# MAPieschl/PointCloudProcessing

Measured on AMD Instinct MI355X. Metric: points/sec PointNet fwd+bwd N=1024 B=32 at 1/2/4/8 MI355X vs CPU ref, higher is better.
Workload: dtype bf16; 1 GPU; PointNet-cls training step (fwd + losses + bwd + grad all-reduce + Adam), N=1024 points, batch 32 per GPU, profile classification_pretrain, 23 classes / 12 parts, random-init weights; global_batch=32, points_per_cloud=1024, parallelism=dp1, launch=hipgraph

## Files before the change

include/pointnet_hip.h:

```cpp
#ifndef POINTNET_HIP_H
#define POINTNET_HIP_H

#include <stddef.h>
#include <stdint.h>

#ifdef __cplusplus
extern "C" {
#endif

#define PN_ABI_VERSION 6

typedef enum {
  PN_OK = 0,
  PN_ERR_INVALID_ARGUMENT = -1,
  PN_ERR_LAUNCH = -2,
  PN_ERR_UNSUPPORTED = -3,
  PN_ERR_WORKSPACE = -4
} pn_status;

#define PN_PREC_BF16 1
#define PN_PREC_BF16X3 3
#define PN_STORE_BF16 0x100
#define PN_IO_KEEP_ACTIVATIONS 1

// ... 25 lines not shown

int pn_conv_fwd_max(const pn_operand* x, const float* w, int B, int N, int K, int C, const float* sgn,
                    float* pmax, int32_t* pidx, float* stat_partials, int prec, pn_stream stream);

int pn_weights_prep(const float* w, const float* sgn, int K, int C, void* wf_hi, void* wf_lo, pn_stream stream);
int pn_panel_slots_per_cloud(int B, int N);
int pn_conv_fwd_max_panel(const pn_operand* x, const void* wf_hi, const void* wf_lo, int B, int N, int K, int C, float* pmax,
                          int32_t* pblock, float* sumsq, int64_t* colacc, int prec, pn_stream stream);
int pn_panel_finalize(const float* pmax, const int32_t* pblock, const float* sumsq, const int64_t* colacc, const void* wf_hi, const void* wf_lo,
                      int prec, int B, int N, int K, int C, const float* gamma, const float* beta, float* moving_mean, float* moving_var,
                      float momentum, float eps, int use_batch_stats, int update_moving, float* mean, float* invstd, float* scale, float* shift,
                      float* g, float* zstar, int32_t* arg_block, pn_stream stream);
int pn_chain_fwd_max(const pn_operand* x, const float* xyz, const float* w1, const void* w1t, const float* scale1, const float* shift1,
                     const void* w2t, const float* scale2, const float* shift2, const void* wf_hi, int B, int N, float* pmax,
                     int32_t* pblock, pn_stream stream);
int pn_weights_copy16(const float* w, int K, int C, void* w16, void* wt16, pn_stream stream);

int pn_max_resolve(const pn_operand* x, const void* wf_hi, const void* wf_lo, const int32_t* arg_block, int B, int N, int K, int C,
                   int32_t* arg, int prec, pn_stream stream);

int pn_maxbwd_scatter(const int32_t* arg, const float* hs, const float* wt, const float* q, int B, int N, int K, int C, float* D, int store16,
                      pn_stream stream);

int pn_conv_bwd_data(const pn_operand* dz, const float* w, int64_t w_cloud_stride, int B, int N, int K, int C,
                     const float* addend, const float* zmask, const float* msc, const float* msh, float* out,
                     float* stat_partials, int prec, pn_stream stream);

int pn_conv_bwd_data_wgrad(const pn_operand* dz, const float* w, int64_t w_cloud_stride, int B, int N, int K, int C,
                           const float* addend, const float* zmask, const float* msc, const float* msh, float* out,
                           float* stat_partials, const pn_operand* a, int Ci, int slab_rows, float* slabs, int prec, pn_stream stream);

int pn_conv_wgrad(const pn_operand* a, const pn_operand* b, int B, int N, int Ci, int Cj, int slab_rows,
                  float* slabs, int prec, pn_stream stream);

int pn_slab_reduce(const float* slabs, int n_slabs, int per_group, int64_t elems, float* out, pn_stream stream);

int pn_bn_finalize(const float* stat_partials, int n_tiles, int C, int64_t count, const float* gamma,
                   const float* beta, float* moving_mean, float* moving_var, float momentum, float eps,
                   int use_batch_stats, int update_moving, float* mean, float* invstd, float* scale, float* shift,
                   pn_stream stream);

int pn_bn_bwd_finalize(const float* stat_partials, int n_tiles, int C, int64_t count, const float* gamma,
                       const float* mean, const float* invstd, int batch_stats, float* dgamma, float* dbeta,
                       float* ca, float* cb, float* cc, pn_stream stream);

int pn_sign(const float* gamma, int C, float* sgn, pn_stream stream);

int pn_max_finalize(const float* pmax, const int32_t* pidx, int B, int tiles_per_cloud, int C, const float* sgn,
                    const float* scale, const float* shift, float* g, float* zstar, int32_t* arg, pn_stream stream);

size_t pn_dense_workspace_floats(int R, int K, int C);
int pn_dense_layer(const float* x, int ldx, const float* w, int ldw, int trans, int R, int K, int C, float* workspace,
                   uint32_t* counters, const float* bias, const float* gamma, const float* beta, float* moving_mean,
                   float* moving_var, float momentum, float eps, int bn_mode, int act, const uint8_t* keep, float keep_scale,
                   float* z_out, float* a_out, float* mean_out, float* invstd_out, pn_stream stream);

int pn_dense_bwd(const float* da, const float* z, const float* x, int ldx, int R, int K, int C, const float* gamma,
                 const float* beta, const float* mean, const float* invstd, int bn_mode, int act, const uint8_t* keep,
                 float keep_scale, float* dz, float* dgamma, float* dbeta, float* dbias, float* dw, pn_stream stream);

typedef struct pn_dense_tail {
  const float *z, *gamma, *beta, *mean, *invstd;
  const uint8_t* keep; float keep_scale;
  int bn_mode, act;
  float *dz, *dgamma, *dbeta, *dbias;
} pn_dense_tail;
// ... 218 lines not shown
```

pointcloudprocessing_amd/_lib.py:

```python
from __future__ import annotations

import ctypes as C
import os
import subprocess

_HERE = os.path.dirname(os.path.abspath(__file__))
LIB_PATH = os.path.join(_HERE, "libpointnet_hip.so")
CSRC = os.path.join(_HERE, "csrc")

PN_PREC_BF16 = 1
PN_PREC_BF16X3 = 3
PN_STORE_BF16 = 0x100
PN_IO_KEEP_ACTIVATIONS = 1
ABI_VERSION = 6
PN_NUM_BLOCKS = 15
PN_ICP_BVH_LEAF = 4
PN_ICP_BVH_MAX_DEPTH = 32
PN_ICP_BVH_PAD_ULPS = 16
PREC = {"bf16": PN_PREC_BF16 | PN_STORE_BF16, "bf16_f32act": PN_PREC_BF16, "bf16x3": PN_PREC_BF16X3}

BLOCK_NAMES = ["input_transform", "mlp_1_1", "mlp_1_2", "feature_transform", "mlp_2_1", "mlp_2_2", "mlp_2_3",
               "mlp_cls_1", "mlp_cls_2", "mlp_cls_3", "mlp_seg_1", "mlp_seg_2", "mlp_seg_3", "mlp_seg_4",
               "mlp_seg_5"]

# ... 40 lines not shown
                ("bwd_phase", C.c_int32), ("flags", C.c_int32), ("dropout_seed", C.c_uint64), ("dropout_step", C.c_void_p),
                ("sync_rank", C.c_int32), ("pad3_", C.c_int32), ("sync_hook", C.c_void_p), ("sync_ctx", C.c_void_p)]


SYNC_HOOK = C.CFUNCTYPE(C.c_int, C.c_void_p, C.c_int, C.c_void_p, C.c_void_p, C.c_int64, C.c_int, C.c_void_p)


_P = C.c_void_p
_I = C.c_int
_I64 = C.c_int64
_F = C.c_float
_D = C.c_double
_OP = C.POINTER(pn_operand)
_DESC = C.POINTER(pn_model_desc)
_IO = C.POINTER(pn_model_io)
SIGNATURES = {
    "pn_abi_version": (_I, []),
    "pn_last_error": (C.c_char_p, []),
    "pn_normalize": (_I, [_P, _I, _I, _P, _P, _P, _P]),
    "pn_conv3_fwd": (_I, [_P, _P, _I64, _I, _I, _I, _P, _P, _P]),
    "pn_conv3_wgrad": (_I, [_P, _OP, _I, _I, _I, _P, _P]),
    "pn_conv_fwd": (_I, [_OP, _P, _I64, _I, _I, _I, _I, _P, _P, _P, _I, _P]),
    "pn_conv_fwd_max": (_I, [_OP, _P, _I, _I, _I, _I, _P, _P, _P, _P, _I, _P]),
    "pn_weights_prep": (_I, [_P, _P, _I, _I, _P, _P, _P]),
    "pn_panel_slots_per_cloud": (_I, [_I, _I]),
    "pn_conv_fwd_max_panel": (_I, [_OP, _P, _P, _I, _I, _I, _I, _P, _P, _P, _P, _I, _P]),
    "pn_panel_finalize": (_I, [_P, _P, _P, _P, _P, _P, _I, _I, _I, _I, _I, _P, _P, _P, _P, _F, _F, _I, _I, _P, _P, _P, _P, _P, _P, _P, _P]),
    "pn_chain_fwd_max": (_I, [_OP, _P, _P, _P, _P, _P, _P, _P, _P, _P, _I, _I, _P, _P, _P]),
    "pn_weights_copy16": (_I, [_P, _I, _I, _P, _P, _P]),
    "pn_max_resolve": (_I, [_OP, _P, _P, _P, _I, _I, _I, _I, _P, _I, _P]),
    "pn_maxbwd_scatter": (_I, [_P, _P, _P, _P, _I, _I, _I, _I, _P, _I, _P]),
    "pn_conv_bwd_data": (_I, [_OP, _P, _I64, _I, _I, _I, _I, _P, _P, _P, _P, _P, _P, _I, _P]),
    "pn_conv_wgrad": (_I, [_OP, _OP, _I, _I, _I, _I, _I, _P, _I, _P]),
    "pn_conv_bwd_data_wgrad": (_I, [_OP, _P, _I64, _I, _I, _I, _I, _P, _P, _P, _P, _P, _P, _OP, _I, _I, _P, _I, _P]),
    "pn_slab_reduce": (_I, [_P, _I, _I, _I64, _P, _P]),
    "pn_bn_finalize": (_I, [_P, _I, _I, _I64, _P, _P, _P, _P, _F, _F, _I, _I, _P, _P, _P, _P, _P]),
    "pn_bn_bwd_finalize": (_I, [_P, _I, _I, _I64, _P, _P, _P, _I, _P, _P, _P, _P, _P, _P]),
    "pn_sign": (_I, [_P, _I, _P, _P]),
    "pn_max_finalize": (_I, [_P, _P, _I, _I, _I, _P, _P, _P, _P, _P, _P, _P]),
    "pn_dense_workspace_floats": (C.c_size_t, [_I, _I, _I]),
    "pn_dense_layer": (_I, [_P, _I, _P, _I, _I, _I, _I, _I, _P, _P, _P, _P, _P, _P, _P, _F, _F, _I, _I, _P, _F, _P, _P, _P, _P, _P]),
    "pn_dense_bwd_step": (_I, [_P, _I, _P, _I, _I, _I, _I, _P, _P, _P, _P, _P]),
    "pn_dense_wgrad_batch": (_I, [_P, _I, _P]),
    "pn_dense_bwd": (_I, [_P, _P, _P, _I, _I, _I, _I, _P, _P, _P, _P, _I, _I, _P, _F, _P, _P, _P, _P, _P, _P]),
    "pn_softmax_xent": (_I, [_P, _I, _I, _P, _F, _P, _P, _P, _P, _P]),
    "pn_argmax_rows": (_I, [_P, _I64, _I, _P, _P]),
    "pn_seg_out_part_stride": (_I, []),
    "pn_seg_out_part_rows": (_I, []),
    "pn_seg_out_fwd": (_I, [_OP, _P, _P, _I64, _I, _I, _P, _F, _P, _P, _P, _P]),
    "pn_bmm": (_I, [_P, _P, _I, _I, _I, _P, _I, _P]),
    "pn_dropout_masks": (_I, [_P, _I64, _P, _I64, _F, C.c_uint64, _P, _P]),
    "pn_count_nonfinite": (_I, [_P, _I64, _I, _P, _P]),
    "pn_fps_workspace_bytes": (C.c_size_t, [_I, _I]),
    "pn_fps": (_I, [_P, _I, _I, _I, _I, _P, _P, _P, C.c_size_t, _P]),
    "pn_voxel_workspace_bytes": (C.c_size_t, [_I]),
    "pn_voxel_downsample": (_I, [_P, _P, _I, C.POINTER(C.c_float), C.POINTER(C.c_float), _I, _P, _P, _P, _P, _P,
                                 C.c_size_t, _P]),
    "pn_knn_propagate": (_I, [_P, _P, _I, _I, _I, _I, _P, _I, _P, _P, _P, _P, _P]),
    "pn_icp_workspace_bytes": (C.c_size_t, [_I, _I, _I, _I]),
    "pn_icp_correspond": (_I, [_P, _P, _I, _I, _P, C.POINTER(C.c_int32), _I, _I, _P, _F, _P, _P, _P, _P, C.c_size_t, _P]),
    "pn_icp_solve": (_I, [_P, _I, _P, _P, _P, _P]),
    "pn_semantic_icp": (_I, [_P, _P, _I, _I, _P, C.POINTER(C.c_int32), _I, _I, _P, _I, _F, _D, _D, _P, _P, _P, _P, _P, _P,
                             C.c_size_t, _P]),
    "pn_icp_normals": (_I, [_P, C.POINTER(C.c_int32), _I, _I, _I, _P, _P, _P, _P]),
    "pn_icp_plane_workspace_bytes": (C.c_size_t, [_I, _I, _I, _I]),
    "pn_icp_plane_sums": (_I, [_P, _P, _I, _I, _P, C.POINTER(C.c_int32), _I, _I, _P, _F, _P, _P, _P, _P, _P, _P, C.c_size_t, _P]),
# ... 123 lines not shown
```

pointcloudprocessing_amd/csrc/pn_api.hip:

```cpp
#include <stdarg.h>
#include "pn_internal.h"

namespace pn {
static thread_local char g_err[512] = "";
void set_error(const char* fmt, ...) {
  va_list ap;
  va_start(ap, fmt);
  vsnprintf(g_err, sizeof(g_err), fmt, ap);
  va_end(ap);
}
const char* get_error() { return g_err; }
}

using namespace pn;
static inline hipStream_t S(pn_stream s) { return reinterpret_cast<hipStream_t>(s); }

extern "C" {

int pn_abi_version(void) { return PN_ABI_VERSION; }
const char* pn_last_error(void) { return get_error(); }

int pn_normalize(const float* xyz, int B, int N, float* out, float* centroid, float* scale, pn_stream stream) {
  return normalize(xyz, B, N, out, centroid, scale, S(stream));
}
// ... 25 lines not shown
                      float* g, float* zstar, int32_t* arg_block, pn_stream stream) {
  return panel_finalize(pmax, pblock, sumsq, reinterpret_cast<const long long*>(colacc), wf_hi, wf_lo, prec, B, N, K, C, gamma, beta, moving_mean, moving_var, momentum, eps,
                        use_batch_stats, update_moving, mean, invstd, scale, shift, g, zstar, arg_block, S(stream));
}
int pn_chain_fwd_max(const pn_operand* x, const float* xyz, const float* w1, const void* w1t, const float* scale1, const float* shift1,
                     const void* w2t, const float* scale2, const float* shift2, const void* wf_hi, int B, int N, float* pmax, int32_t* pblock,
                     pn_stream stream) {
  return chain_fwd_max(x, xyz, w1, w1t, scale1, shift1, w2t, scale2, shift2, wf_hi, B, N, pmax, pblock, S(stream));
}
int pn_weights_copy16(const float* w, int K, int C, void* w16, void* wt16, pn_stream stream) { return weights_copy16(w, K, C, w16, wt16, S(stream)); }
int pn_max_resolve(const pn_operand* x, const void* wf_hi, const void* wf_lo, const int32_t* arg_block, int B, int N, int K, int C,
                   int32_t* arg, int prec, pn_stream stream) {
  return max_resolve(x, wf_hi, wf_lo, prec, arg_block, B, N, K, C, arg, S(stream));
}
int pn_maxbwd_scatter(const int32_t* arg, const float* hs, const float* wt, const float* q, int B, int N, int K, int C, float* D, int store16,
                      pn_stream stream) {
  PN_CHECK_ARG(B > 0 && N > 0 && C > 0, "pn_maxbwd_scatter: bad sizes");
  return maxbwd_scatter(arg, hs, wt, q, B, N, K, C, D, store16, S(stream));
}
int pn_conv_bwd_data(const pn_operand* dz, const float* w, int64_t wcs, int B, int N, int K, int C, const float* addend,
                     const float* zmask, const float* msc, const float* msh, float* out, float* part, int prec, pn_stream stream) {
  return conv_bwd_data(dz, w, wcs, B, N, K, C, addend, zmask, msc, msh, out, part, prec, S(stream));
}
int pn_conv_bwd_data_wgrad(const pn_operand* dz, const float* w, int64_t wcs, int B, int N, int K, int C, const float* addend,
                           const float* zmask, const float* msc, const float* msh, float* out, float* part, const pn_operand* a, int Ci,
                           int slab_rows, float* slabs, int prec, pn_stream stream) {
  PN_CHECK_ARG(a != nullptr, "pn_conv_bwd_data_wgrad: null operand a");
  const WgradFuse wf{*a, Ci, slab_rows, slabs};
  return conv_bwd_data(dz, w, wcs, B, N, K, C, addend, zmask, msc, msh, out, part, prec, S(stream), nullptr, nullptr, &wf);
}
int pn_conv_wgrad(const pn_operand* a, const pn_operand* b, int B, int N, int Ci, int Cj, int slab_rows, float* slabs, int prec,
                  pn_stream stream) {
  return conv_wgrad(a, b, B, N, Ci, Cj, slab_rows, slabs, prec, S(stream));
}
int pn_slab_reduce(const float* slabs, int n_slabs, int per_group, int64_t elems, float* out, pn_stream stream) {
  return slab_reduce(slabs, n_slabs, per_group, elems, out, S(stream));
}
int pn_bn_finalize(const float* part, int n_tiles, int C, int64_t count, const float* gamma, const float* beta, float* mm, float* mv,
                   float momentum, float eps, int use_batch_stats, int update_moving, float* mean, float* invstd, float* scale,
                   float* shift, pn_stream stream) {
  return bn_finalize(part, n_tiles, C, count, gamma, beta, mm, mv, momentum, eps, use_batch_stats, update_moving, mean, invstd, scale,
                     shift, S(stream));
}
int pn_bn_bwd_finalize(const float* part, int n_tiles, int C, int64_t count, const float* gamma, const float* mean,
                       const float* invstd, int batch_stats, float* dgamma, float* dbeta, float* ca, float* cb, float* cc,
                       pn_stream stream) {
  return bn_bwd_finalize(part, n_tiles, C, count, gamma, mean, invstd, batch_stats, dgamma, dbeta, ca, cb, cc, S(stream));
}
int pn_sign(const float* gamma, int C, float* sgn, pn_stream stream) { return sign_of(gamma, C, sgn, S(stream)); }
int pn_max_finalize(const float* pmax, const int32_t* pidx, int B, int tpc, int C, const float* sgn, const float* scale,
                    const float* shift, float* g, float* zstar, int32_t* arg, pn_stream stream) {
  return max_finalize(pmax, pidx, B, tpc, C, 0x7fffffff, sgn, scale, shift, g, zstar, arg, S(stream));
}
size_t pn_dense_workspace_floats(int R, int K, int C) { return dense_partial_floats(R, K, C); }
int pn_dense_layer(const float* x, int ldx, const float* w, int ldw, int trans, int R, int K, int C, float* workspace, uint32_t* counters,
                   const float* bias, const float* gamma, const float* beta, float* moving_mean, float* moving_var, float momentum,
                   float eps, int bn_mode, int act, const uint8_t* keep, float keep_scale, float* z_out, float* a_out, float* mean_out,
                   float* invstd_out, pn_stream stream) {
  return dense_layer(x, ldx, w, ldw, trans != 0, R, K, C, workspace, counters, bias, gamma, beta, moving_mean, moving_var, momentum, eps,
                     bn_mode, act, keep, keep_scale, z_out, a_out, mean_out, invstd_out, S(stream));
}
int pn_dense_bwd(const float* da, const float* z, const float* x, int ldx, int R, int K, int C, const float* gamma, const float* beta,
                 const float* mean, const float* invstd, int bn_mode, int act, const uint8_t* keep, float keep_scale, float* dz,
                 float* dgamma, float* dbeta, float* dbias, float* dw, pn_stream stream) {
  if (R <= 32)
    return dense_bwd_fused(da, z, x, ldx, R, K, C, gamma, beta, mean, invstd, bn_mode, act, keep, keep_scale, dz, dgamma, dbeta, dbias, dw,
// ... 194 lines not shown
```

pointcloudprocessing_amd/csrc/pn_gemm.hip:

```cpp
#include <vector>
#include "pn_common.h"
#include "pn_dense_wgrad.h"
#include "pn_gemm_core.h"
#include "pn_internal.h"
#include "pn_slab_reduce.h"

namespace pn {

template <int BM, int BN, int NS, bool B2>
__global__ __launch_bounds__(256) void wgrad_batch_kernel(const WgradBatch wb) {
  __shared__ __attribute__((aligned(16))) unsigned char lds_raw[GemmLds<BM, BN, NS>::BYTES];
  wgrad_batch_tile<BM, BN, NS, B2>(wb, (int)blockIdx.x, lds_raw);
}

template <int BM, int BN, int NS, bool B2>
__global__ __launch_bounds__(256) void wgrad_batch_dense_kernel(const WgradBatch wb, int n_w, const DenseWgradBatch db) {
  __shared__ __attribute__((aligned(16))) unsigned char lds_raw[GemmLds<BM, BN, NS>::BYTES];
  static_assert(GemmLds<BM, BN, NS>::BYTES >= 16 * 32 * 4, "the dense riders' LDS tile fits");
  if ((int)blockIdx.x >= n_w) {
    dense_wgrad_batch_body(db, (int)blockIdx.x - n_w, reinterpret_cast<float(*)[32]>(lds_raw));
    return;
  }
  wgrad_batch_tile<BM, BN, NS, B2>(wb, (int)blockIdx.x, lds_raw);
}

struct WgLds {
  static constexpr int PITCH = Geo<64>::PITCH;
  static constexpr int W = 2 * 128 * PITCH, A = W + 64 * PITCH, RED_BYTES = (A + 128 * PITCH) * 2, BYTES = RED_BYTES + 4 * 64 * 4;
  static_assert(BYTES <= 65536, "the fused weight-gradient tile's LDS exceeds the static __shared__ limit");
};
template <int BM, int BN, int NS, int MODE, bool A2, int EPI, bool ADD, bool MASK, bool AH, bool S16, bool W16 = false, bool WG = false>
__device__ __forceinline__ void rows_tile_t(const GemmArgs& g, const int bx, const int by, unsigned char* lds_raw, const WgArgs* wa = nullptr) {
  constexpr int BK = (NS == 3) ? 32 : 64;
  constexpr int PITCH = Geo<BK>::PITCH;
  constexpr int MT = BM / 64, NT = BN / 64;
  constexpr int WTM = BM / 2, WTN = BN / 2;
  constexpr int TILE_A = BM * PITCH, TILE_B = BN * PITCH;
  static_assert(!WG || (BM == 128 && BN == 64 && NS == 1 && MODE == MODE_BWD && EPI == EPI_STORE && AH && S16), "the fused weight-gradient tile");
  __bf16* Ahi = reinterpret_cast<__bf16*>(lds_raw);
  __bf16* Bhi = Ahi + (WG ? WgLds::W : TILE_A);
  __bf16* Alo = (NS == 3) ? (Bhi + TILE_B) : Ahi;
  __bf16* Blo = (NS == 3) ? (Alo + TILE_A) : Bhi;

  const int tid = threadIdx.x, lane = tid & 63, wave = tid >> 6;
  const int wm = wave >> 1, wn = wave & 1;
  const int wrow0 = wm * WTM, wcol0 = wn * WTN;

  f32x16 acc[MT][NT];
#pragma unroll
  for (int m = 0; m < MT; ++m)
#pragma unroll
    for (int n = 0; n < NT; ++n)
#pragma unroll
      for (int e = 0; e < 16; ++e) acc[m][n][e] = 0.f;

  const int cloud = bx / g.tiles_per_cloud, tin = bx - cloud * g.tiles_per_cloud;

  const int row_in_cloud0 = tin * BM;
  const int nrows = min(BM, g.N - row_in_cloud0);
  const long long row0 = (long long)cloud * g.N + row_in_cloud0;
  const int col0 = by * BN;
  const long long wbase = (long long)cloud * g.w_cloud_stride;
  pn_operand wop;
  wop.s1 = g.w; wop.s2 = nullptr; wop.ca = nullptr; wop.cb = nullptr; wop.cc = nullptr;
  wop.lo = -INFINITY; wop.h16 = 0;
  wop.ld = (MODE == MODE_FWD) ? g.C : g.K;

  NatStage<BM, BK, A2, AH> sa;
  TrnStage<BN, BK, false, false> sbT;
  NatStage<BN, BK, false, false> sbN;
  CopyStage<BN, BK> sbC;
  auto issue_chunk = [&](int k0) {
    if (!(g.dbg & 4)) sa.issue(g.a, row0 * g.a.ld, nrows, k0, tid);
    if constexpr (W16) {
      sbC.issue(g.w16, (long long)col0 * g.K, g.K, g.C - col0, k0, tid);
    } else if (MODE == MODE_FWD) {
      if (!(g.dbg & 8)) sbT.issue(wop, wbase + (long long)k0 * g.C + col0, BK, g.C - col0, tid);
    } else {
      sbN.issue(wop, wbase + (long long)col0 * g.K, g.C - col0, k0, tid);
    }
  };
  NatStage<BM, BK, false, true> swg;
  if constexpr (WG) swg.issue(wa->a, row0 * wa->a.ld, nrows, 0, tid);
  if (g.K > 0) issue_chunk(0);
  for (int k0 = 0; k0 < g.K; k0 += BK) {
    sa.pin();
    if constexpr (WG) {
      Ahi = reinterpret_cast<__bf16*>(lds_raw) + (k0 / BK) * TILE_A;
      Alo = Ahi;
    }
    sa.template finish<NS>(Ahi, Alo, g.a, nrows, k0, tid);
    if constexpr (W16) {
      sbC.pin();
      sbC.finish(Bhi, g.C - col0, tid);
    } else if (MODE == MODE_FWD) {
      sbT.pin();
      sbT.template finish<NS>(Bhi, Blo, wop, BK, g.C - col0, 0, tid);
    } else {
      sbN.pin();
      sbN.template finish<NS>(Bhi, Blo, wop, g.C - col0, k0, tid);
    }
    __syncthreads();
    if (k0 + BK < g.K) issue_chunk(k0 + BK);
    mma_chunk<MT, NT, BK, NS>(acc, Ahi, Alo, Bhi, Blo, wrow0, wcol0, lane);
    __syncthreads();
  }
  if constexpr (WG) {
    swg.pin();
    swg.template finish<1>(reinterpret_cast<__bf16*>(lds_raw) + WgLds::A, reinterpret_cast<__bf16*>(lds_raw) + WgLds::A, wa->a, nrows, 0, tid);
  }

  const int r = lane & 31, h = lane >> 5;
  const bool full = (nrows == BM) && (col0 + BN <= g.C);
  float* red = reinterpret_cast<float*>(lds_raw + (WG ? WgLds::RED_BYTES : 0));

  if (EPI == EPI_STORE) {
    float s1[NT], s2[NT];
#pragma unroll
    for (int n = 0; n < NT; ++n) {
      const int jl = wcol0 + n * 32 + r, j = col0 + jl;
      const bool jv = j < g.C;
      float bias = 0.f, msc = 0.f, msh = 0.f;
      if (jv && g.cloud_bias) bias = g.cloud_bias[(long long)cloud * g.cloud_bias_stride + j];
      if (jv && g.zmask) { msc = g.msc[j]; msh = g.msh[j]; }
      float a1 = 0.f, a2 = 0.f;
#pragma unroll
      for (int m = 0; m < MT; ++m) {
        const int il0 = wrow0 + m * 32 + 4 * h;
        if (full) {
          if (g.out && !(g.dbg & 1)) epi_store_block<true, ADD, MASK, true, S16>(acc[m][n], g, row0, il0, nrows, j, jv, bias, msc, msh, a1, a2);
          else epi_store_block<true, ADD, MASK, false, S16>(acc[m][n], g, row0, il0, nrows, j, jv, bias, msc, msh, a1, a2);
        } else {
          if (g.out) epi_store_block<false, ADD, MASK, true, S16>(acc[m][n], g, row0, il0, nrows, j, jv, bias, msc, msh, a1, a2);
          else epi_store_block<false, ADD, MASK, false, S16>(acc[m][n], g, row0, il0, nrows, j, jv, bias, msc, msh, a1, a2);
        }
      }
      s1[n] = a1 + __shfl_xor(a1, 32, 64);
      s2[n] = a2 + __shfl_xor(a2, 32, 64);
// ... 92 lines not shown
    const int ncol = g.ncol;
    if (ncol > 1) {
      const int lin = blockIdx.x, nrow = (int)gridDim.x / ncol, full = (nrow / 8) * 8 * ncol;
      if (lin < full) {
        const int grp = lin / (8 * ncol), r = lin - grp * 8 * ncol;
        by = r >> 3;
        bx = grp * 8 + (r & 7);
      } else {
        const int l2 = lin - full, rem = nrow - (nrow / 8) * 8;
        bx = (nrow / 8) * 8 + l2 % rem;
        by = l2 / rem;
      }
    }
    if (g.a.h16) {
      if constexpr (NS == 1 && EPI == EPI_STORE) {
        if (g.w16) {
          if (g.store16) rows_tile_t<BM, BN, NS, MODE, A2, EPI, ADD, MASK, true, true, true>(g, bx, by, lds_raw);
          else rows_tile_t<BM, BN, NS, MODE, A2, EPI, ADD, MASK, true, false, true>(g, bx, by, lds_raw);
          return;
        }
      }
      if (EPI == EPI_STORE && g.store16) rows_tile_t<BM, BN, NS, MODE, A2, EPI, ADD, MASK, true, EPI == EPI_STORE>(g, bx, by, lds_raw);
      else rows_tile_t<BM, BN, NS, MODE, A2, EPI, ADD, MASK, true, false>(g, bx, by, lds_raw);
    } else {
      if (EPI == EPI_STORE && g.store16) rows_tile_t<BM, BN, NS, MODE, A2, EPI, ADD, MASK, false, EPI == EPI_STORE>(g, bx, by, lds_raw);
      else rows_tile_t<BM, BN, NS, MODE, A2, EPI, ADD, MASK, false, false>(g, bx, by, lds_raw);
    }
  }
}

template <bool ADD, bool MASK>
__global__ __launch_bounds__(256) void gemm_bwd_wgrad_kernel(const GemmArgs g, const WgArgs wa) {
  __shared__ __attribute__((aligned(16))) unsigned char lds_raw[WgLds::BYTES];
  if (g.w16) rows_tile_t<128, 64, 1, MODE_BWD, true, EPI_STORE, ADD, MASK, true, true, true, true>(g, (int)blockIdx.x, 0, lds_raw, &wa);
  else rows_tile_t<128, 64, 1, MODE_BWD, true, EPI_STORE, ADD, MASK, true, true, false, true>(g, (int)blockIdx.x, 0, lds_raw, &wa);
}

template <bool AH, bool S16>
__global__ __launch_bounds__(256) void gemm_bwd_reduce_kernel(const GemmArgs g, int n_gemm, const float* __restrict__ slabs, int per_group,
                                                              long long elems, float* __restrict__ red_out, int nb_per_group) {
  constexpr int LDS_BYTES = (128 + 64) * Geo<64>::PITCH * 2;
  static_assert(LDS_BYTES >= 8 * 32 * 4, "the riders' LDS tile fits");
  __shared__ __attribute__((aligned(16))) unsigned char lds_raw[LDS_BYTES];
  if ((int)blockIdx.x >= n_gemm) {
    const int bx = (int)blockIdx.x - n_gemm;
    slab_reduce_block(slabs, per_group, elems, red_out, bx % nb_per_group, bx / nb_per_group, reinterpret_cast<float(*)[32]>(lds_raw));
    return;
  }
  rows_tile_t<128, 64, 1, MODE_BWD, false, EPI_STORE, false, false, AH, S16>(g, (int)blockIdx.x, 0, lds_raw);
}

template <int BM, int BN, int NS, int MODE, bool A2, bool B2, int EPI, bool ADD = false, bool MASK = false>
static int launch(const GemmArgs& g, dim3 grid, hipStream_t st) {
  hipLaunchKernelGGL((gemm_kernel<BM, BN, NS, MODE, A2, B2, EPI, ADD, MASK>), grid, dim3(256), 0, st, g);
  PN_CHECK_LAUNCH();
  return PN_OK;
}

static bool aligned16(const void* p) { return (reinterpret_cast<uintptr_t>(p) & 15) == 0; }

static int check_operand(const pn_operand* o, const char* name) {
  PN_CHECK_ARG(o && o->s1, "%s: null operand", name);
  PN_CHECK_ARG(aligned16(o->s1) && (!o->s2 || aligned16(o->s2)), "%s: s1/s2 must be 16-byte aligned", name);
  PN_CHECK_ARG((!o->ca || aligned16(o->ca)) && (!o->cb || aligned16(o->cb)) && (!o->cc || aligned16(o->cc)),
               "%s: coefficient vectors must be 16-byte aligned", name);
  PN_CHECK_ARG(o->ld > 0 && o->ld % 4 == 0, "%s: ld must be a positive multiple of 4", name);
  PN_CHECK_ARG(o->h16 == 0 || (o->h16 == 1 && o->ld % 8 == 0), "%s: h16 must be 0 or 1, and 16-bit rows need ld %% 8 == 0", name);
  return PN_OK;
// ... 65 lines not shown
  PN_CHECK_ARG(K >= 64 && K % 64 == 0, "pn_conv_fwd_max: K must be a multiple of 64 (K=%d)", K);
  PN_CHECK_ARG(C >= 128 && C % 128 == 0, "pn_conv_fwd_max: C must be a multiple of 128 (C=%d)", C);
  PN_CHECK_ARG(x->ld >= K, "pn_conv_fwd_max: x.ld < K");
  PN_CHECK_ARG(w && aligned16(w) && sgn && pmax && pidx, "pn_conv_fwd_max: null pointer");
  PN_CHECK_ARG(prec == PN_PREC_BF16 || prec == PN_PREC_BF16X3, "pn_conv_fwd_max: bad prec %d", prec);
  GemmArgs g;
  memset(&g, 0, sizeof(g));
  g.a = *x; g.w = w; g.B = B; g.N = N; g.K = K; g.C = C;
  g.tiles_per_cloud = cdiv(N, 128);
  g.sgn = sgn; g.pmax = pmax; g.pidx = pidx; g.stat_partials = stat_partials;
  return dispatch_rows<MODE_FWD, false, EPI_MAX>(g, prec, st);
}

int conv_bwd_data(const pn_operand* dz, const float* w, long long wcs, int B, int N, int K, int C, const float* addend,
                  const float* zmask, const float* msc, const float* msh, float* out, float* stat_partials, int prec,
                  hipStream_t st, const void* w16, const float* col_bias, const WgradFuse* wf) {
  PN_TRY(check_operand(dz, "pn_conv_bwd_data.dz"));
  PN_CHECK_ARG(B > 0 && N > 0, "pn_conv_bwd_data: B and N must be positive");
  PN_CHECK_ARG(K >= 64 && K % 64 == 0, "pn_conv_bwd_data: K must be a multiple of 64 (K=%d)", K);
  PN_CHECK_ARG(C >= 64 && C % 64 == 0, "pn_conv_bwd_data: C must be a multiple of 64 (C=%d)", C);
  PN_CHECK_ARG(dz->ld >= K, "pn_conv_bwd_data: dz.ld < K");
  PN_CHECK_ARG(w && aligned16(w), "pn_conv_bwd_data: w null or unaligned");
  PN_CHECK_ARG(!zmask || (msc && msh), "pn_conv_bwd_data: zmask needs msc and msh");
  const int store16 = (prec & PN_STORE_BF16) ? 1 : 0;
  prec &= ~PN_STORE_BF16;
  PN_CHECK_ARG(prec == PN_PREC_BF16 || prec == PN_PREC_BF16X3, "pn_conv_bwd_data: bad prec %d", prec);
  GemmArgs g;
  memset(&g, 0, sizeof(g));
  g.store16 = store16;
  g.a = *dz; g.w = w; g.w_cloud_stride = wcs; g.B = B; g.N = N; g.K = K; g.C = C;
  g.tiles_per_cloud = cdiv(N, 128);
  g.out = out; g.addend = addend; g.zmask = zmask; g.msc = msc; g.msh = msh; g.stat_partials = stat_partials;
  g.cloud_bias = col_bias; g.cloud_bias_stride = 0;
  if (w16 && wcs == 0 && prec == PN_PREC_BF16 && dz->h16 && (reinterpret_cast<uintptr_t>(w16) & 15) == 0 && K % 8 == 0)
    g.w16 = reinterpret_cast<const unsigned short*>(w16);
  if (wf) {
    PN_TRY(check_operand(&wf->a, "pn_conv_bwd_data_wgrad.a"));
    PN_CHECK_ARG(prec == PN_PREC_BF16 && store16 && dz->h16 && dz->s2, "pn_conv_bwd_data_wgrad: bf16 operands, bf16 storage and a two-source dz");
    PN_CHECK_ARG(C == 64 && (K == 64 || K == 128), "pn_conv_bwd_data_wgrad: C must be 64 and K 64 or 128 (C=%d K=%d)", C, K);
    PN_CHECK_ARG(wf->Ci == C && wf->a.h16 && !wf->a.s2 && wf->a.ld >= wf->Ci, "pn_conv_bwd_data_wgrad: operand a must be a 64-channel bf16 single-source operand");
    PN_CHECK_ARG(wf->slab_rows == 64 || wf->slab_rows == 128, "pn_conv_bwd_data_wgrad: slab_rows must be 64 or 128 (%d)", wf->slab_rows);
    PN_CHECK_ARG(wf->slabs != nullptr, "pn_conv_bwd_data_wgrad: null slabs");
    const WgArgs wa{wf->a, wf->slabs, wf->slab_rows};
    g.ncol = 1;
    const dim3 grid(B * g.tiles_per_cloud);
    const bool ha = addend != nullptr, hm = zmask != nullptr;
    if (ha && hm) hipLaunchKernelGGL((gemm_bwd_wgrad_kernel<true, true>), grid, dim3(256), 0, st, g, wa);
    else if (ha) hipLaunchKernelGGL((gemm_bwd_wgrad_kernel<true, false>), grid, dim3(256), 0, st, g, wa);
    else if (hm) hipLaunchKernelGGL((gemm_bwd_wgrad_kernel<false, true>), grid, dim3(256), 0, st, g, wa);
    else hipLaunchKernelGGL((gemm_bwd_wgrad_kernel<false, false>), grid, dim3(256), 0, st, g, wa);
    PN_CHECK_LAUNCH();
    return PN_OK;
  }
  if (dz->s2) return dispatch_bwd<true>(g, prec, st);
  return dispatch_bwd<false>(g, prec, st);
}

int conv_bwd_data_reduce(const pn_operand* dz, const float* w, long long wcs, int B, int N, int K, int C, float* out, int prec, hipStream_t st,
                         const float* slabs, int n_slabs, int per_group, long long elems, float* red_out, bool* rode) {
  *rode = false;
  PN_TRY(check_operand(dz, "pn_conv_bwd_data.dz"));
  PN_CHECK_ARG(B > 0 && N > 0 && w && aligned16(w) && out && dz->ld >= K, "conv_bwd_data_reduce: bad arguments");
  PN_CHECK_ARG(slabs && red_out && n_slabs > 0 && per_group > 0 && n_slabs % per_group == 0 && elems > 0, "conv_bwd_data_reduce: bad sizes");
  const int store16 = (prec & PN_STORE_BF16) ? 1 : 0;
  prec &= ~PN_STORE_BF16;
  const long long nb = cdivll(elems, 32), riders = nb * (n_slabs / per_group), n_gemm = (long long)B * cdiv(N, 128);
// ... 153 lines not shown
```

pointcloudprocessing_amd/csrc/pn_gemm_core.h:

```cpp
#pragma once
#include "pn_common.h"
#include "pn_internal.h"

namespace pn {

typedef __attribute__((ext_vector_type(8))) __bf16 bf16x8;
typedef __attribute__((ext_vector_type(16))) float f32x16;

enum { MODE_FWD = 0, MODE_BWD = 1, MODE_WGRAD = 2 };
enum { EPI_STORE = 0, EPI_MAX = 1, EPI_SLAB = 2 };

struct GemmArgs {
  pn_operand a;
  pn_operand b;
  const float* w;
  const unsigned short* w16;
  long long w_cloud_stride;
  int B, N;
  int K;
  int C;
  int Ci;
  int tiles_per_cloud;
  float* out;
  const float* cloud_bias;
  long long cloud_bias_stride;
  const float* addend;
  const float* zmask;
  const float* msc;
  const float* msh;
  float* stat_partials;
  const float* sgn;
  float* pmax;
  int* pidx;
  int store16;
  int ncol;
  int colsum;
  int dbg;
};
struct WgArgs {
  pn_operand a;
  float* slabs;
  int rows;
};

template <int BK>
struct Geo {
  static constexpr int PITCH = BK + 8;
};

__device__ __forceinline__ void cvt_store8(__bf16* hi, __bf16* lo, const float (&v)[8], bool split) {
  bf16x8 h;
#pragma unroll
  for (int e = 0; e < 8; ++e) h[e] = (__bf16)v[e];
  *reinterpret_cast<bf16x8*>(hi) = h;
  if (split) {
    bf16x8 l;
#pragma unroll
    for (int e = 0; e < 8; ++e) l[e] = (__bf16)(v[e] - (float)h[e]);
    *reinterpret_cast<bf16x8*>(lo) = l;
  }
}


template <int TR, int BK, bool HAS2, bool H16>
struct NatStage {
  static constexpr int CH = BK / 8;
  static constexpr int RP = 256 / CH;
  static constexpr int P = TR / RP;
  static constexpr int Q = H16 ? 1 : 2;
  float4 x[P][Q];
  float4 y[HAS2 ? P : 1][Q];

  __device__ __forceinline__ void issue(const pn_operand& op, long long base, int nvalid_rows, int k0, int tid) {
    const int ch = tid % CH, rin = tid / CH;
    const int k = k0 + ch * 8;
#pragma unroll
    for (int p = 0; p < P; ++p) {
      const int r = p * RP + rin;
      const long long rr = (r < nvalid_rows) ? r : (nvalid_rows - 1);
      if constexpr (H16) {
        x[p][0] = __builtin_bit_cast(float4, act_load8_raw(op.s1, base + rr * op.ld + k));
        if (HAS2) y[p][0] = __builtin_bit_cast(float4, act_load8_raw(op.s2, base + rr * op.ld + k));
      } else {
        const float* s = op.s1 + base + rr * op.ld + k;
        x[p][0] = *reinterpret_cast<const float4*>(s);
        x[p][1] = *reinterpret_cast<const float4*>(s + 4);
        if (HAS2) {
          const float* s2 = op.s2 + base + rr * op.ld + k;
          y[p][0] = *reinterpret_cast<const float4*>(s2);
          y[p][1] = *reinterpret_cast<const float4*>(s2 + 4);
        }
      }
    }
  }
  __device__ __forceinline__ void pin() {
#pragma unroll
    for (int p = 0; p < P; ++p)
#pragma unroll
      for (int q = 0; q < Q; ++q) {
        asm volatile("" : "+v"(x[p][q].x), "+v"(x[p][q].y), "+v"(x[p][q].z), "+v"(x[p][q].w));
        if (HAS2) asm volatile("" : "+v"(y[p][q].x), "+v"(y[p][q].y), "+v"(y[p][q].z), "+v"(y[p][q].w));
      }
  }
  template <int NS>
  __device__ __forceinline__ void finish(__bf16* __restrict__ Thi, __bf16* __restrict__ Tlo, const pn_operand& op,
                                         int nvalid_rows, int k0, int tid) {
    constexpr int PITCH = Geo<BK>::PITCH;
    const int ch = tid % CH, rin = tid / CH;
    const int k = k0 + ch * 8;
    float ca[8], cb[8], cc[8];
#pragma unroll
    for (int e = 0; e < 8; ++e) { ca[e] = 1.f; cb[e] = 0.f; cc[e] = 0.f; }
    if (op.ca) {
      const float4 t0 = *reinterpret_cast<const float4*>(op.ca + k), t1 = *reinterpret_cast<const float4*>(op.ca + k + 4);
      ca[0] = t0.x; ca[1] = t0.y; ca[2] = t0.z; ca[3] = t0.w; ca[4] = t1.x; ca[5] = t1.y; ca[6] = t1.z; ca[7] = t1.w;
    }
    if (HAS2 && op.cb) {
      const float4 t0 = *reinterpret_cast<const float4*>(op.cb + k), t1 = *reinterpret_cast<const float4*>(op.cb + k + 4);
      cb[0] = t0.x; cb[1] = t0.y; cb[2] = t0.z; cb[3] = t0.w; cb[4] = t1.x; cb[5] = t1.y; cb[6] = t1.z; cb[7] = t1.w;
    }
    if (op.cc) {
      const float4 t0 = *reinterpret_cast<const float4*>(op.cc + k), t1 = *reinterpret_cast<const float4*>(op.cc + k + 4);
      cc[0] = t0.x; cc[1] = t0.y; cc[2] = t0.z; cc[3] = t0.w; cc[4] = t1.x; cc[5] = t1.y; cc[6] = t1.z; cc[7] = t1.w;
    }
    const float lo = op.lo;
#pragma unroll
    for (int p = 0; p < P; ++p) {
      const int r = p * RP + rin;
      const bool rv = r < nvalid_rows;
      float v[8], w[8];
      if constexpr (H16) {
        bf16x8_unpack(__builtin_bit_cast(uint4, x[p][0]), v);
        if (HAS2) bf16x8_unpack(__builtin_bit_cast(uint4, y[p][0]), w);
      } else {
        v[0] = x[p][0].x; v[1] = x[p][0].y; v[2] = x[p][0].z; v[3] = x[p][0].w;
        v[4] = x[p][Q - 1].x; v[5] = x[p][Q - 1].y; v[6] = x[p][Q - 1].z; v[7] = x[p][Q - 1].w;
        if (HAS2) {
          w[0] = y[p][0].x; w[1] = y[p][0].y; w[2] = y[p][0].z; w[3] = y[p][0].w;
          w[4] = y[p][Q - 1].x; w[5] = y[p][Q - 1].y; w[6] = y[p][Q - 1].z; w[7] = y[p][Q - 1].w;
        }
      }
#pragma unroll
      for (int e = 0; e < 8; ++e) {
        float t = fmaf(ca[e], v[e], cc[e]);
        if (HAS2) t = fmaf(cb[e], w[e], t);
        v[e] = rv ? clamp_lo(t, lo) : 0.f;
      }
      cvt_store8(Thi + r * PITCH + ch * 8, Tlo + r * PITCH + ch * 8, v, NS == 3);
    }
  }
};

template <int TR, int BK, bool HAS2, bool H16>
struct TrnStage {
  static constexpr int KG = BK / 8;
  static constexpr int TRL = H16 ? TR / 2 : TR;
  static constexpr int TPG = 256 / TRL;
// ... 409 lines not shown
```

Before: 47.08 million points/s.

## Issue both K chunks ahead in fused bwd-data+wgrad GEMM for short K

For the fused data-gradient/weight-gradient kernel with K at most two chunks, global loads for both K chunks (including BN coefficient loads) are issued up front in separate register stages before any LDS staging and MMA. This exposes more memory-level parallelism and hides load latency that the serial issue-one-ahead loop left exposed. It costs extra registers per thread, which may reduce occupancy. The path is gated by a PN_LOAD_AHEAD env var that defaults on, and a colsum wgrad API entry point is also added.

```diff
diff --git a/include/pointnet_hip.h b/include/pointnet_hip.h
--- a/include/pointnet_hip.h
+++ b/include/pointnet_hip.h
@@ -81,6 +81,8 @@
 
 int pn_conv_wgrad(const pn_operand* a, const pn_operand* b, int B, int N, int Ci, int Cj, int slab_rows,
                   float* slabs, int prec, pn_stream stream);
+int pn_conv_wgrad_colsum(const pn_operand* a, const pn_operand* b, int B, int N, int Ci, int Cj, int slab_rows,
+                         float* slabs, int prec, pn_stream stream);
 
 int pn_slab_reduce(const float* slabs, int n_slabs, int per_group, int64_t elems, float* out, pn_stream stream);
 
diff --git a/pointcloudprocessing_amd/_lib.py b/pointcloudprocessing_amd/_lib.py
--- a/pointcloudprocessing_amd/_lib.py
+++ b/pointcloudprocessing_amd/_lib.py
@@ -96,6 +96,7 @@
     "pn_maxbwd_scatter": (_I, [_P, _P, _P, _P, _I, _I, _I, _I, _P, _I, _P]),
     "pn_conv_bwd_data": (_I, [_OP, _P, _I64, _I, _I, _I, _I, _P, _P, _P, _P, _P, _P, _I, _P]),
     "pn_conv_wgrad": (_I, [_OP, _OP, _I, _I, _I, _I, _I, _P, _I, _P]),
+    "pn_conv_wgrad_colsum": (_I, [_OP, _OP, _I, _I, _I, _I, _I, _P, _I, _P]),
     "pn_conv_bwd_data_wgrad": (_I, [_OP, _P, _I64, _I, _I, _I, _I, _P, _P, _P, _P, _P, _P, _OP, _I, _I, _P, _I, _P]),
     "pn_slab_reduce": (_I, [_P, _I, _I, _I64, _P, _P]),
     "pn_bn_finalize": (_I, [_P, _I, _I, _I64, _P, _P, _P, _P, _F, _F, _I, _I, _P, _P, _P, _P, _P]),
diff --git a/pointcloudprocessing_amd/csrc/pn_api.hip b/pointcloudprocessing_amd/csrc/pn_api.hip
--- a/pointcloudprocessing_amd/csrc/pn_api.hip
+++ b/pointcloudprocessing_amd/csrc/pn_api.hip
@@ -81,6 +81,10 @@
 int pn_conv_wgrad(const pn_operand* a, const pn_operand* b, int B, int N, int Ci, int Cj, int slab_rows, float* slabs, int prec,
                   pn_stream stream) {
   return conv_wgrad(a, b, B, N, Ci, Cj, slab_rows, slabs, prec, S(stream));
+}
+int pn_conv_wgrad_colsum(const pn_operand* a, const pn_operand* b, int B, int N, int Ci, int Cj, int slab_rows, float* slabs, int prec,
+                         pn_stream stream) {
+  return conv_wgrad(a, b, B, N, Ci, Cj, slab_rows, slabs, prec, S(stream), 1);
 }
 int pn_slab_reduce(const float* slabs, int n_slabs, int per_group, int64_t elems, float* out, pn_stream stream) {
   return slab_reduce(slabs, n_slabs, per_group, elems, out, S(stream));
diff --git a/pointcloudprocessing_amd/csrc/pn_gemm.hip b/pointcloudprocessing_amd/csrc/pn_gemm.hip
--- a/pointcloudprocessing_amd/csrc/pn_gemm.hip
+++ b/pointcloudprocessing_amd/csrc/pn_gemm.hip
@@ -7,6 +7,10 @@
 
 namespace pn {
 
+static int load_ahead() {
+  static const int v = getenv("PN_LOAD_AHEAD") ? atoi(getenv("PN_LOAD_AHEAD")) : 1;
+  return v != 0;
+}
 template <int BM, int BN, int NS, bool B2>
 __global__ __launch_bounds__(256) void wgrad_batch_kernel(const WgradBatch wb) {
   __shared__ __attribute__((aligned(16))) unsigned char lds_raw[GemmLds<BM, BN, NS>::BYTES];
@@ -29,7 +33,43 @@
   static constexpr int W = 2 * 128 * PITCH, A = W + 64 * PITCH, RED_BYTES = (A + 128 * PITCH) * 2, BYTES = RED_BYTES + 4 * 64 * 4;
   static_assert(BYTES <= 65536, "the fused weight-gradient tile's LDS exceeds the static __shared__ limit");
 };
-template <int BM, int BN, int NS, int MODE, bool A2, int EPI, bool ADD, bool MASK, bool AH, bool S16, bool W16 = false, bool WG = false>
+template <int BM, int BN, int BK, int NS, int MODE, bool A2, bool AH, bool W16>
+struct RowChunk {
+  NatStage<BM, BK, A2, AH> sa;
+  TrnStage<BN, BK, false, false> sbT;
+  NatStage<BN, BK, false, false> sbN;
+  CopyStage<BN, BK> sbC;
+  float ca[8], cb[8], cc[8];
+  __device__ __forceinline__ void issue(const GemmArgs& g, const pn_operand& wop, long long row0, int nrows, int col0, long long wbase, int k0, int tid) {
+    NatStage<BM, BK, A2, AH>::coef_load(g.a, k0, tid, ca, cb, cc);
+    sa.issue(g.a, row0 * g.a.ld, nrows, k0, tid);
+    if constexpr (W16) {
+      sbC.issue(g.w16, (long long)col0 * g.K, g.K, g.C - col0, k0, tid);
+    } else if (MODE == MODE_FWD) {
+      sbT.issue(wop, wbase + (long long)k0 * g.C + col0, BK, g.C - col0, tid);
+    } else {
+      sbN.issue(wop, wbase + (long long)col0 * g.K, g.C - col0, k0, tid);
+    }
+  }
+  __device__ __forceinline__ void stage(__bf16* Ahi, __bf16* Alo, __bf16* Bhi, __bf16* Blo, const GemmArgs& g, const pn_operand& wop, int nrows,
+                                        int col0, int k0, int tid) {
+    sa.pin();
+    sa.template finish_c<NS>(Ahi, Alo, g.a, nrows, tid, ca, cb, cc);
+    if constexpr (W16) {
+      sbC.pin();
+      sbC.finish(Bhi, g.C - col0, tid);
+    } else if (MODE == MODE_FWD) {
+      sbT.pin();
+      sbT.template finish<NS>(Bhi, Blo, wop, BK, g.C - col0, 0, tid);
+    } else {
+      sbN.pin();
+      sbN.template finish<NS>(Bhi, Blo, wop, g.C - col0, k0, tid);
+    }
+  }
+};
+
+template <int BM, int BN, int NS, int MODE, bool A2, int EPI, bool ADD, bool MASK, bool AH, bool S16, bool W16 = false, bool WG = false,
+          bool LA = false>
 __device__ __forceinline__ void rows_tile_t(const GemmArgs& g, const int bx, const int by, unsigned char* lds_raw, const WgArgs* wa = nullptr) {
   constexpr int BK = (NS == 3) ? 32 : 64;
   constexpr int PITCH = Geo<BK>::PITCH;
@@ -82,28 +122,52 @@
   };
   NatStage<BM, BK, false, true> swg;
   if constexpr (WG) swg.issue(wa->a, row0 * wa->a.ld, nrows, 0, tid);
-  if (g.K > 0) issue_chunk(0);
-  for (int k0 = 0; k0 < g.K; k0 += BK) {
-    sa.pin();
-    if constexpr (WG) {
-      Ahi = reinterpret_cast<__bf16*>(lds_raw) + (k0 / BK) * TILE_A;
-      Alo = Ahi;
-    }
-    sa.template finish<NS>(Ahi, Alo, g.a, nrows, k0, tid);
-    if constexpr (W16) {
-      sbC.pin();
-      sbC.finish(Bhi, g.C - col0, tid);
-    } else if (MODE == MODE_FWD) {
-      sbT.pin();
-      sbT.template finish<NS>(Bhi, Blo, wop, BK, g.C - col0, 0, tid);
-    } else {
-      sbN.pin();
-      sbN.template finish<NS>(Bhi, Blo, wop, g.C - col0, k0, tid);
-    }
-    __syncthreads();
-    if (k0 + BK < g.K) issue_chunk(k0 + BK);
-    mma_chunk<MT, NT, BK, NS>(acc, Ahi, Alo, Bhi, Blo, wrow0, wcol0, lane);
-    __syncthreads();
+  static_assert(!LA || (NS == 1 && MODE == MODE_BWD), "the load-ahead form is built for the bf16 data-gradient GEMMs");
+  if (LA && g.ahead && g.K <= 2 * BK) {
+    RowChunk<BM, BN, BK, NS, MODE, A2, AH, W16> c0, c1;
+    const bool two = g.K > BK;
+    if (g.K > 0) c0.issue(g, wop, row0, nrows, col0, wbase, 0, tid);
+    if (two) c1.issue(g, wop, row0, nrows, col0, wbase, BK, tid);
+    if (g.K > 0) {
+      c0.stage(Ahi, Alo, Bhi, Blo, g, wop, nrows, col0, 0, tid);
+      __syncthreads();
+      mma_chunk<MT, NT, BK, NS>(acc, Ahi, Alo, Bhi, Blo, wrow0, wcol0, lane);
+      __syncthreads();
+    }
+    if (two) {
+      if constexpr (WG) {
+        Ahi = reinterpret_cast<__bf16*>(lds_raw) + TILE_A;
+        Alo = Ahi;
+      }
+      c1.stage(Ahi, Alo, Bhi, Blo, g, wop, nrows, col0, BK, tid);
+      __syncthreads();
+      mma_chunk<MT, NT, BK, NS>(acc, Ahi, Alo, Bhi, Blo, wrow0, wcol0, lane);
+      __syncthreads();
+    }
+  } else {
+    if (g.K > 0) issue_chunk(0);
+    for (int k0 = 0; k0 < g.K; k0 += BK) {
+      sa.pin();
+      if constexpr (WG) {
+        Ahi = reinterpret_cast<__bf16*>(lds_raw) + (k0 / BK) * TILE_A;
+        Alo = Ahi;
+      }
+      sa.template finish<NS>(Ahi, Alo, g.a, nrows, k0, tid);
+      if constexpr (W16) {
+        sbC.pin();
+        sbC.finish(Bhi, g.C - col0, tid);
+      } else if (MODE == MODE_FWD) {
+        sbT.pin();
+        sbT.template finish<NS>(Bhi, Blo, wop, BK, g.C - col0, 0, tid);
+      } else {
+        sbN.pin();
+        sbN.template finish<NS>(Bhi, Blo, wop, g.C - col0, k0, tid);
+      }
+      __syncthreads();
+      if (k0 + BK < g.K) issue_chunk(k0 + BK);
+      mma_chunk<MT, NT, BK, NS>(acc, Ahi, Alo, Bhi, Blo, wrow0, wcol0, lane);
+      __syncthreads();
+    }
   }
   if constexpr (WG) {
     swg.pin();
@@ -262,8 +326,8 @@
 template <bool ADD, bool MASK>
 __global__ __launch_bounds__(256) void gemm_bwd_wgrad_kernel(const GemmArgs g, const WgArgs wa) {
   __shared__ __attribute__((aligned(16))) unsigned char lds_raw[WgLds::BYTES];
-  if (g.w16) rows_tile_t<128, 64, 1, MODE_BWD, true, EPI_STORE, ADD, MASK, true, true, true, true>(g, (int)blockIdx.x, 0, lds_raw, &wa);
-  else rows_tile_t<128, 64, 1, MODE_BWD, true, EPI_STORE, ADD, MASK, true, true, false, true>(g, (int)blockIdx.x, 0, lds_raw, &wa);
+  if (g.w16) rows_tile_t<128, 64, 1, MODE_BWD, true, EPI_STORE, ADD, MASK, true, true, true, true, true>(g, (int)blockIdx.x, 0, lds_raw, &wa);
+  else rows_tile_t<128, 64, 1, MODE_BWD, true, EPI_STORE, ADD, MASK, true, true, false, true, true>(g, (int)blockIdx.x, 0, lds_raw, &wa);
 }
 
 template <bool AH, bool S16>
@@ -395,6 +459,7 @@
   g.tiles_per_cloud = cdiv(N, 128);
   g.out = out; g.addend = addend; g.zmask = zmask; g.msc = msc; g.msh = msh; g.stat_partials = stat_partials;
   g.cloud_bias = col_bias; g.cloud_bias_stride = 0;
+  g.ahead = load_ahead();
   if (w16 && wcs == 0 && prec == PN_PREC_BF16 && dz->h16 && (reinterpret_cast<uintptr_t>(w16) & 15) == 0 && K % 8 == 0)
     g.w16 = reinterpret_cast<const unsigned short*>(w16);
   if (wf) {
diff --git a/pointcloudprocessing_amd/csrc/pn_gemm_core.h b/pointcloudprocessing_amd/csrc/pn_gemm_core.h
--- a/pointcloudprocessing_amd/csrc/pn_gemm_core.h
+++ b/pointcloudprocessing_amd/csrc/pn_gemm_core.h
@@ -36,6 +36,7 @@
   int ncol;
   int colsum;
   int dbg;
+  int ahead;
 };
 struct WgArgs {
   pn_operand a;
@@ -102,13 +103,8 @@
         if (HAS2) asm volatile("" : "+v"(y[p][q].x), "+v"(y[p][q].y), "+v"(y[p][q].z), "+v"(y[p][q].w));
       }
   }
-  template <int NS>
-  __device__ __forceinline__ void finish(__bf16* __restrict__ Thi, __bf16* __restrict__ Tlo, const pn_operand& op,
-                                         int nvalid_rows, int k0, int tid) {
-    constexpr int PITCH = Geo<BK>::PITCH;
-    const int ch = tid % CH, rin = tid / CH;
-    const int k = k0 + ch * 8;
-    float ca[8], cb[8], cc[8];
+  static __device__ __forceinline__ void coef_load(const pn_operand& op, int k0, int tid, float (&ca)[8], float (&cb)[8], float (&cc)[8]) {
+    const int k = k0 + (tid % CH) * 8;
 #pragma unroll
     for (int e = 0; e < 8; ++e) { ca[e] = 1.f; cb[e] = 0.f; cc[e] = 0.f; }
     if (op.ca) {
@@ -123,6 +119,19 @@
       const float4 t0 = *reinterpret_cast<const float4*>(op.cc + k), t1 = *reinterpret_cast<const float4*>(op.cc + k + 4);
       cc[0] = t0.x; cc[1] = t0.y; cc[2] = t0.z; cc[3] = t0.w; cc[4] = t1.x; cc[5] = t1.y; cc[6] = t1.z; cc[7] = t1.w;
     }
+  }
+  template <int NS>
+  __device__ __forceinline__ void finish(__bf16* __restrict__ Thi, __bf16* __restrict__ Tlo, const pn_operand& op,
+                                         int nvalid_rows, int k0, int tid) {
+    float ca[8], cb[8], cc[8];
+    coef_load(op, k0, tid, ca, cb, cc);
+    finish_c<NS>(Thi, Tlo, op, nvalid_rows, tid, ca, cb, cc);
+  }
+  template <int NS>
+  __device__ __forceinline__ void finish_c(__bf16* __restrict__ Thi, __bf16* __restrict__ Tlo, const pn_operand& op, int nvalid_rows, int tid,
+                                           const float (&ca)[8], const float (&cb)[8], const float (&cc)[8]) {
+    constexpr int PITCH = Geo<BK>::PITCH;
+    const int ch = tid % CH, rin = tid / CH;
     const float lo = op.lo;
 #pragma unroll
     for (int p = 0; p < P; ++p) {
```

Result: faster. 47.96 million points/s, median of 6 (+1.9%).
